# pachyderm-io/pfs

Hardware: AMD Instinct MI355X
Metric: GiB/s device-resident CDC rolling-hash + chunk content-hash (higher is better)
Workload: dtype u8

## Files before the change

### pfs_amd/csrc/cdc_kernels.hip

```cpp
#include <hip/hip_runtime.h>
#include <stdint.h>
#include <stdlib.h>

#include <algorithm>
#include <type_traits>

#define PFSCDC_HD __host__ __device__
#include "index_parse.h"
#include "pfscdc_internal.h"

#define PFS_DEV __device__ __forceinline__

namespace pfscdc {


PFS_DEV uint64_t rotl1_64(uint64_t x) { return (x << 1) | (x >> 63); }

PFS_DEV uint32_t tab_addr(uint32_t w, uint32_t lane_off, int j) {
  return __builtin_amdgcn_perm(w, lane_off, 0x0c0c0000u | ((4u + (uint32_t)j) << 8));
}

template <typename T>
PFS_DEV T lds_load(const uint8_t* lds, uint32_t byte_addr) {
  return *reinterpret_cast<const T*>(lds + byte_addr);
// ... 614 lines not shown
    }
    uint64_t total;
    const uint64_t ex = block_exscan<BLOCK>(e, s_wave, &total) + carry;
    if (t < ntiles) {
      const uint64_t ts = t * kTile;
      if (c <= (uint32_t)kTileK) {
        uint32_t o[kTileK];
#pragma unroll
        for (int i = 0; i < kTileK; i++) o[i] = i < (int)c ? recs[t].off[i] : ~0u;
#pragma unroll
        for (int i = 0; i < kTileK; i++) {
          uint32_t rank = 0;
#pragma unroll
          for (int j = 0; j < kTileK; j++) rank += o[j] < o[i];
          if (i < (int)c) entries[ex + rank] = ts + o[i];
        }
      } else {
        const uint64_t te = (ts + kTile < n) ? ts + kTile : n;
        entries[ex] = kDenseBit | (te - 1);
      }
    }
    carry += total;
  }
  if (threadIdx.x == 0) *n_entries = carry;
}

__global__ __launch_bounds__(kCompactBlock) void compact_kernel(
    const TileRec* __restrict__ recs, uint64_t ntiles, uint64_t n,
    uint64_t* __restrict__ entries, uint64_t* __restrict__ n_entries) {
  __shared__ uint64_t s_wave[kCompactBlock / 64 + 1];
  compact_tiles<kCompactBlock>(recs, ntiles, n, entries, n_entries, s_wave);
}

template <int BLOCK>
PFS_DEV uint64_t segcompact_block(const pfscdc_segment* __restrict__ slots,
                                  const uint64_t* __restrict__ seg_base,
                                  const uint64_t* __restrict__ nseg, uint32_t nfiles,
                                  pfscdc_segment* __restrict__ segs,
                                  uint64_t* __restrict__ seg_begin, uint64_t* s_wave) {
  uint64_t carry = 0;
  for (uint64_t base = 0; base < nfiles; base += BLOCK) {
    const uint64_t f = base + threadIdx.x;
    const uint64_t c = f < nfiles ? nseg[f] : 0;
    uint64_t total;
    const uint64_t ex = block_exscan<BLOCK>(c, s_wave, &total) + carry;
    if (f < nfiles) {
      seg_begin[f] = ex;
      const pfscdc_segment* src = slots + seg_base[f];
      for (uint64_t i = 0; i < c; i++) segs[ex + i] = src[i];
    }
    carry += total;
  }
  if (threadIdx.x == 0) seg_begin[nfiles] = carry;
  return carry;
}

PFS_DEV uint32_t lpt_key(uint64_t size) {
  const uint64_t nblk = (size + 127) / 128;
  const uint64_t k = nblk >> 6;
  return 1023u - (uint32_t)(k < 1023 ? k : 1023);
}

template <int BLOCK>
PFS_DEV void lpt_order_block(const pfscdc_segment* __restrict__ segs, uint64_t n,
                             uint32_t* __restrict__ order, uint32_t* __restrict__ counter,
                             uint32_t* hist, uint64_t* s_wave,
                             const uint64_t* __restrict__ offs = nullptr, uint64_t bin_bytes = 0,
                             uint32_t* __restrict__ next = nullptr, uint64_t* qlen = nullptr) {
  const bool bins = next && offs && bin_bytes;
  auto binned = [&](uint64_t i) {
    const uint32_t f = segs[i].file;
    return bins && offs[f + 1] - offs[f] <= bin_bytes;
  };
  auto entry = [&](uint64_t i, uint32_t& key) {
    if (binned(i)) {
      const uint32_t f = segs[i].file;
      key = lpt_key(offs[f + 1] - offs[f]);
      return i == 0 || segs[i - 1].file != f;
    }
    key = lpt_key(segs[i].size);
    return true;
  };
  constexpr int kPer = 1024 / BLOCK;
  static_assert(1024 % BLOCK == 0, "bins split evenly over the block");
  for (int b = 0; b < kPer; b++) hist[threadIdx.x * kPer + b] = 0;
  __syncthreads();
  for (uint64_t i = threadIdx.x; i < n; i += BLOCK) {
    uint32_t key;
    if (entry(i, key)) atomicAdd(&hist[key], 1u);
    if (bins) next[i] = binned(i) && i + 1 < n && segs[i + 1].file == segs[i].file
                            ? (uint32_t)(i + 1) : kNoNext;
  }
  __syncthreads();
  uint32_t local[kPer];
  uint64_t sum = 0;
  for (int b = 0; b < kPer; b++) {
    local[b] = hist[threadIdx.x * kPer + b];
    sum += local[b];
  }
  uint64_t total;
  uint64_t start = block_exscan<BLOCK>(sum, s_wave, &total);
  for (int b = 0; b < kPer; b++) {
    hist[threadIdx.x * kPer + b] = (uint32_t)start;
    start += local[b];
  }
  __syncthreads();
  for (uint64_t i = threadIdx.x; i < n; i += BLOCK) {
    uint32_t key;
    if (entry(i, key)) order[atomicAdd(&hist[key], 1u)] = (uint32_t)i;
  }
  if (threadIdx.x == 0) {
    *counter = 0;
    if (qlen) *qlen = total;
  }
}


PFS_DEV uint64_t rescan_first(const uint8_t* __restrict__ data, const uint64_t* __restrict__ T,
                              uint64_t a, uint64_t b, uint64_t mask) {
  const uint32_t lane = threadIdx.x & 63u;
  constexpr uint64_t W = 256;
  for (uint64_t base = a; base <= b; base += 64 * W) {
    const uint64_t st = base + lane * W;
    const uint64_t en = (st + W - 1 < b) ? st + W - 1 : b;
    uint64_t found = kNone;
    if (st <= en) {
      uint64_t h = 0;
      for (int k = 0; k < 64; k++) h = rotl1_64(h) ^ T[data[st - 63 + k]];
      if ((h & mask) == 0) found = st;
      for (uint64_t i = st + 1; found == kNone && i <= en; i++) {
        h = rotl1_64(h) ^ T[data[i - 64]] ^ T[data[i]];
        if ((h & mask) == 0) found = i;
      }
    }
    found = wave_min_u64(found);
    if (found != kNone) return found;
  }
  return kNone;
}

PFS_DEV void select_file(
    const uint8_t* __restrict__ data, const uint64_t* __restrict__ T,
    const uint64_t* __restrict__ entries, const uint64_t* __restrict__ n_entries,
    const uint64_t* __restrict__ offs, const uint64_t* __restrict__ seg_base, uint64_t f,
    uint64_t mask, uint64_t min_chunk, uint64_t max_chunk,
    pfscdc_segment* __restrict__ slots, uint64_t* __restrict__ nseg) {
  const uint32_t lane = threadIdx.x & 63u;
  const uint64_t fs = offs[f], fe = offs[f + 1];
  const uint64_t sb = seg_base[f], cap = seg_base[f + 1] - sb;
  const uint64_t ne = *n_entries;
  pfscdc_segment* out = slots + sb;
  uint64_t count = 0;
  auto emit = [&](uint64_t s, uint64_t size, uint32_t flags) {
    if (lane == 0 && count < cap) {
      out[count].offset = s - fs;
      out[count].size = size;
      out[count].file = (uint32_t)f;
      out[count].flags = flags;
    }
    count++;
  };
  uint64_t k = 0;
  {
    const uint64_t key = fs + min_chunk - 1;
    uint64_t lo = 0, hi = ne;
    while (hi - lo > 64) {
      const uint64_t step = (hi - lo + 63) / 64;
      const uint64_t i = lo + lane * step;
      const bool below = i < hi && (entries[i] & ~kDenseBit) < key;
      const uint32_t cnt = (uint32_t)__popcll(__ballot(below));
      if (cnt == 0) {
        hi = lo;
      } else {
        const uint64_t top = lo + (uint64_t)cnt * step;
        lo = lo + (uint64_t)(cnt - 1) * step + 1;
        hi = top < hi ? top : hi;
      }
    }
    const uint64_t i = lo + lane;
    const bool below = i < hi && (entries[i] & ~kDenseBit) < key;
    k = lo + (uint64_t)__popcll(__ballot(below));
  }
  uint64_t s = fs;
  while (true) {
    const uint64_t lo = s + min_chunk - 1;
    if (lo >= fe) break;
    const uint64_t hi = s + max_chunk - 1;
    const uint64_t limit = hi < fe - 1 ? hi : fe - 1;
    while (k < ne && (entries[k] & ~kDenseBit) < lo) k++;
    uint64_t c = kNone;
    for (uint64_t kk = k; kk < ne; kk++) {
      const uint64_t e = entries[kk];
      const uint64_t v = e & ~kDenseBit;
      if (!(e & kDenseBit)) {
        if (v <= limit) c = v;
        break;
      }
      const uint64_t ts = (v / kTile) * kTile;
      const uint64_t a = lo > ts ? lo : ts;
      const uint64_t bnd = v < limit ? v : limit;
      if (a <= bnd) {
        c = rescan_first(data, T, a, bnd, mask);
        if (c != kNone) break;
      }
      if (v >= limit) break;
    }
    uint64_t cut;
    if (c != kNone) cut = c;
    else if (hi <= fe - 1) cut = hi;
    else break;
    emit(s, cut + 1 - s, PFSCDC_SEG_VALID | PFSCDC_SEG_CUT);
    s = cut + 1;
  }
  if (s < fe) emit(s, fe - s, PFSCDC_SEG_VALID);
  if (lane == 0) {
    for (uint64_t i = count; i < cap; i++) out[i].flags = 0;
    nseg[f] = count;
  }
}

__global__ __launch_bounds__(kSelectBlock) void select_kernel(
    const uint8_t* __restrict__ data, const uint64_t* __restrict__ T,
    const uint64_t* __restrict__ entries, const uint64_t* __restrict__ n_entries,
    const uint64_t* __restrict__ offs, const uint64_t* __restrict__ seg_base, uint32_t nfiles,
    uint64_t mask, uint64_t min_chunk, uint64_t max_chunk,
    pfscdc_segment* __restrict__ slots, uint64_t* __restrict__ nseg, uint32_t* done_ctr,
    pfscdc_segment* __restrict__ segs, uint64_t* __restrict__ seg_begin,
    uint32_t* __restrict__ order, uint32_t* __restrict__ counter, uint64_t bin_bytes,
    uint32_t* __restrict__ next, uint64_t* __restrict__ qlen) {
  __shared__ uint32_t hist[1024];
  __shared__ uint64_t s_wave[kSelectBlock / 64 + 1];
  __shared__ uint32_t s_flag;
  const uint64_t f = ((uint64_t)blockIdx.x * kSelectBlock + threadIdx.x) >> 6;
  if (f < nfiles)
    select_file(data, T, entries, n_entries, offs, seg_base, f, mask, min_chunk, max_chunk,
                slots, nseg);
  if (!last_block_done(done_ctr, &s_flag)) return;
  const uint64_t total = segcompact_block<kSelectBlock>(slots, seg_base, nseg, nfiles, segs,
                                                        seg_begin, s_wave);
  __threadfence_block();
  __syncthreads();
  if (order)
    lpt_order_block<kSelectBlock>(segs, total, order, counter, hist, s_wave, offs, bin_bytes,
                                  next, qlen);
}


__global__ __launch_bounds__(kCompactBlock) void segcompact_kernel(
    const pfscdc_segment* __restrict__ slots, const uint64_t* __restrict__ seg_base,
    const uint64_t* __restrict__ nseg, uint32_t nfiles, pfscdc_segment* __restrict__ segs,
    uint64_t* __restrict__ seg_begin) {
  __shared__ uint64_t s_wave[kCompactBlock / 64 + 1];
  segcompact_block<kCompactBlock>(slots, seg_base, nseg, nfiles, segs, seg_begin, s_wave);
}

__global__ __launch_bounds__(kCompactBlock) void hash_order_kernel(
    const pfscdc_segment* __restrict__ segs, const uint64_t* __restrict__ seg_count,
    uint32_t* __restrict__ order, uint32_t* __restrict__ counter) {
  __shared__ uint32_t hist[1024];
  __shared__ uint64_t s_wave[kCompactBlock / 64 + 1];
  lpt_order_block<kCompactBlock>(segs, *seg_count, order, counter, hist, s_wave);
}


constexpr uint64_t kB2IV[8] = {
    0x6a09e667f3bcc908ULL, 0xbb67ae8584caa73bULL, 0x3c6ef372fe94f82bULL,
    0xa54ff53a5f1d36f1ULL, 0x510e527fade682d1ULL, 0x9b05688c2b3e6c1fULL,
    0x1f83d9abfb41bd6bULL, 0x5be0cd19137e2179ULL};

template <typename T>
PFS_DEV T pick4(uint32_t j, T v0, T v1, T v2, T v3) {
  return j == 0 ? v0 : j == 1 ? v1 : j == 2 ? v2 : v3;
}

constexpr uint32_t kSigmaPack[12][4] = {
#define PK(a, b, c, d) ((uint32_t)(a) * 8u | (uint32_t)(b) * 8u << 8 | (uint32_t)(c) * 8u << 16 | (uint32_t)(d) * 8u << 24)
#define ROW(s0, s1, s2, s3, s4, s5, s6, s7, s8, s9, s10, s11, s12, s13, s14, s15) \
  {PK(s0, s1, s14, s15), PK(s2, s3, s8, s9), PK(s4, s5, s10, s11), PK(s6, s7, s12, s13)}
    ROW(0, 1, 2, 3, 4, 5, 6, 7, 8, 9, 10, 11, 12, 13, 14, 15),
    ROW(14, 10, 4, 8, 9, 15, 13, 6, 1, 12, 0, 2, 11, 7, 5, 3),
    ROW(11, 8, 12, 0, 5, 2, 15, 13, 10, 14, 3, 6, 7, 1, 9, 4),
    ROW(7, 9, 3, 1, 13, 12, 11, 14, 2, 6, 5, 10, 4, 0, 15, 8),
    ROW(9, 0, 5, 7, 2, 4, 10, 15, 14, 1, 11, 12, 6, 8, 3, 13),
    ROW(2, 12, 6, 10, 0, 11, 8, 3, 4, 13, 7, 5, 15, 14, 1, 9),
    ROW(12, 5, 1, 15, 14, 13, 4, 10, 0, 7, 6, 3, 9, 2, 8, 11),
    ROW(13, 11, 7, 14, 12, 1, 3, 9, 5, 0, 15, 4, 8, 6, 2, 10),
    ROW(6, 15, 14, 9, 11, 3, 0, 8, 12, 2, 13, 7, 1, 4, 10, 5),
// ... 1010 lines not shown
  scan_skip_kernel<<<grid, 256, 0, st>>>(offs, nfiles, n, min_chunk, nunits, skip,
                                         (unsigned long long*)scanned, uinfo, plan);
  hipError_t e = hipGetLastError();
  if (e != hipSuccess) return e;
  scan_slots_kernel<<<grid, 256, 0, st>>>(nunits, uinfo, plan, slots, hdr, d_hdr);
  return hipGetLastError();
}

hipError_t launch_scan(const uint8_t* data, const uint8_t* tail, uint64_t n, const uint64_t* d_table,
                       uint32_t average_bits, uint64_t ntiles, TileRec* recs, int grid,
                       uint32_t* unit_ctr, uint32_t* done_ctr, uint64_t* entries,
                       uint64_t* n_entries, uint64_t* span, hipStream_t st, const uint32_t* skip,
                       const ScanPlan* d_plan) {
  const size_t lds = kScanLdsBytes;
  const uint64_t mask64 = average_bits >= 64 ? ~0ULL : ((1ULL << average_bits) - 1);
  const ScanPlan* const pl = d_plan;
  if (average_bits <= 32)
    cdc_scan_kernel<false><<<grid, kScanBlock, lds, st>>>(
        data, tail, n, d_table, 32 - average_bits, mask64, ntiles, recs, unit_ctr, done_ctr,
        entries, n_entries, skip, span, pl);
  else
    cdc_scan_kernel<true><<<grid, kScanBlock, lds, st>>>(
        data, tail, n, d_table, 64 - average_bits, mask64, ntiles, recs, unit_ctr, done_ctr,
        entries, n_entries, skip, span, pl);
  return hipGetLastError();
}

hipError_t launch_compact(const TileRec* recs, uint64_t ntiles, uint64_t n, uint64_t* entries,
                          uint64_t* n_entries, hipStream_t st) {
  compact_kernel<<<1, kCompactBlock, 0, st>>>(recs, ntiles, n, entries, n_entries);
  return hipGetLastError();
}

hipError_t launch_select(const uint8_t* data, const uint64_t* d_table, const uint64_t* entries,
                         const uint64_t* n_entries, const uint64_t* offs,
                         const uint64_t* seg_base, uint32_t nfiles, uint32_t average_bits,
                         uint64_t min_chunk, uint64_t max_chunk, pfscdc_segment* slots,
                         uint64_t* nseg, uint32_t* done_ctr, pfscdc_segment* segs,
                         uint64_t* seg_begin, uint32_t* order, uint32_t* counter,
                         hipStream_t st, uint64_t bin_bytes, uint32_t* next, uint64_t* qlen) {
  const uint64_t mask64 = average_bits >= 64 ? ~0ULL : ((1ULL << average_bits) - 1);
  const uint64_t waves_per_block = kSelectBlock / 64;
  const uint64_t grid = (nfiles + waves_per_block - 1) / waves_per_block;
  select_kernel<<<(unsigned)grid, kSelectBlock, 0, st>>>(data, d_table, entries, n_entries,
                                                         offs, seg_base, nfiles, mask64,
                                                         min_chunk, max_chunk, slots, nseg,
                                                         done_ctr, segs, seg_begin, order,
                                                         counter, bin_bytes, next, qlen);
  return hipGetLastError();
}

hipError_t launch_segcompact(const pfscdc_segment* slots, const uint64_t* seg_base,
                             const uint64_t* nseg, uint32_t nfiles, pfscdc_segment* segs,
                             uint64_t* seg_begin, hipStream_t st) {
  segcompact_kernel<<<1, kCompactBlock, 0, st>>>(slots, seg_base, nseg, nfiles, segs, seg_begin);
  return hipGetLastError();
}

static uint32_t prio_arg(uint32_t prio) {
  return prio == kHashPrioNone ? 0u : prio ? prio : kHashPrioAuto;
}

int hash_waves(uint64_t longest_bytes, uint64_t total_bytes, int num_cus, int forced) {
  if (forced >= 1 && forced <= 8) return forced;
  const uint64_t quads1 = (uint64_t)num_cus * 4 * (64 / 4);
  const uint64_t longest = (longest_bytes + 127) / 128, total = total_bytes / 128;
  return longest * quads1 >= total ? 1 : kHashWavesPerSimd;
}

static unsigned capped_grid(uint64_t grid, Knob cap_knob) {
  const int64_t cap = knob(cap_knob);
  if (cap > 0 && (uint64_t)cap < grid) grid = (uint64_t)cap;
  return (unsigned)grid;
}

static unsigned hash_grid(uint64_t max_segments, int num_cus, int waves) {
  const uint64_t quads_per_block = kHashBlock / 4;
  const uint64_t need = (max_segments + quads_per_block - 1) / quads_per_block;
  const uint64_t full = (uint64_t)num_cus * 4 * (waves > 0 ? waves : kHashWavesPerSimd) /
                        (kHashBlock / 64);
  return capped_grid(need < full ? need : full, Knob::HashGrid);
}

hipError_t launch_blake2b(const uint8_t* data, const uint64_t* offs, pfscdc_segment* segs,
                          const uint64_t* seg_count, uint64_t max_segments, uint32_t* order,
                          uint32_t* counter, int num_cus, uint64_t nbytes, hipStream_t st,
                          bool ordered, uint64_t* span, int waves, uint32_t prio,
                          bool cu_exclusive, const uint32_t* next, uint64_t* fair,
// ... 1393 lines not shown
```

### pfs_amd/csrc/pfscdc.cpp

```cpp
#include <hip/hip_runtime.h>

#include <algorithm>
#include <cstdio>
#include <cstring>
#include <string>
#include <vector>

#include <unistd.h>

#include "dev_list.h"
#include "pfscdc_internal.h"

using namespace pfscdc;

namespace {

template <typename T>
struct DevBuf {
  T* p = nullptr;
  size_t cap = 0;
  hipError_t ensure(size_t n, bool exact = false) {
    if (n <= cap && p) return hipSuccess;
    if (p) (void)hipFree(p);
    p = nullptr;
// ... 34 lines not shown
};

struct CreatePending {
  bool active = false, split = false;
  uint32_t k = 0, nr = 0;
  uint8_t* hashes = nullptr;
  pfscdc_ref* refs = nullptr;
};

}

struct pfscdc_ctx {
  pfscdc_params params{};
  int device = 0;
  int num_cus = 256;
  hipStream_t own_stream = nullptr;
  hipStream_t stream = nullptr;
  std::string err;
  uint64_t table[256];
  uint64_t* d_table = nullptr;
  DevBuf<uint8_t> d_data, d_tail;
  DevBuf<TileRec> d_recs;
  DevBuf<uint32_t> d_unit_ctr;
  DevBuf<uint32_t> d_skip;
  DevBuf<uint32_t> d_uinfo, d_plan;
  DevBuf<uint4> d_uslots;
  DevBuf<uint32_t> d_rslots;
  DevBuf<ScanPlan> d_planhdr;
  bool scan_skipped = false;
  uint32_t scan_mode = 0;
  uint64_t scanned_bytes = 0;
  bool cuts_only = false;
  DevBuf<uint64_t> d_entries, d_counts;
  DevBuf<uint64_t> d_offs, d_seg_base, d_nseg, d_seg_begin;
  DevBuf<pfscdc_segment> d_slots, d_segs;
  DevBuf<uint32_t> d_order, d_qctr;
  DevBuf<uint32_t> d_next;
  DevBuf<pfscdc_ref> d_refs;
  DevBuf<uint8_t> d_out;
  DevBuf<uint64_t> d_span;
  PinnedBuf<uint64_t> h_span;
  double wall_khz = 100000.0;
  DevBuf<uint32_t> d_ids;
  DevBuf<uint64_t> d_starts;
  DevBuf<uint8_t> d_group, d_group_ct;
  DevBuf<pfscdc_segment> d_segs2;
  DevBuf<uint64_t> d_blk;
  DevBuf<uint8_t> d_ctext;
  PinnedBuf<uint64_t> h_blk;
  PinnedBuf<pfscdc_segment> h_segs2;
  PinnedBuf<pfscdc_ref> h_refs;
  DevBuf<pfscdc_slice> d_rslices;
  DevBuf<uint64_t> d_rmeta;
  DevBuf<uint8_t> d_rok;
  PinnedBuf<pfscdc_slice> h_rslices;
  PinnedBuf<uint64_t> h_rmeta;
  PinnedBuf<uint8_t> h_rok;
  DevBuf<TarEntry> d_tar;
  DevBuf<uint8_t> d_tnames;
  PinnedBuf<TarEntry> h_tar;
  PinnedBuf<uint8_t> h_tnames;
  hipEvent_t rev[4] = {nullptr, nullptr, nullptr, nullptr};
  float read_ms[2] = {0.f, 0.f};
  float frame_ms = 0.f;
  uint32_t options = 0;
  float get_ms = 0.f;
// ... 397 lines not shown
  if (!file_offsets) return fail(c, PFSCDC_EINVAL, "file_offsets is NULL");
  if (nbytes && !bytes) return fail(c, PFSCDC_EINVAL, "bytes is NULL");
  if (file_offsets[0] != 0 || file_offsets[nfiles] != nbytes)
    return fail(c, PFSCDC_EINVAL, "file_offsets must start at 0 and end at nbytes");
  for (uint32_t f = 0; f < nfiles; f++)
    if (file_offsets[f + 1] < file_offsets[f])
      return fail(c, PFSCDC_EINVAL, "file_offsets must be nondecreasing");
  if (bytes_on_device && ((uintptr_t)bytes & 15))
    return fail(c, PFSCDC_EINVAL, "device bytes must be 16-byte aligned");
  c->ntiles = (nbytes + kTile - 1) / kTile;
  if (c->ntiles * (uint64_t)kScanWaves >= (1ull << 32))
    return fail(c, PFSCDC_EUNSUPPORTED, "batch too large for one scan (split it)");
  c->scan_valid = false;
  HIP_OK(c, hipSetDevice(c->device));
  hipStream_t st = c->stream;
  const pfscdc_params& p = c->params;

  HIP_OK(c, c->h_offs.ensure(nfiles + 1));
  HIP_OK(c, c->h_seg_base.ensure(nfiles + 1));
  std::memcpy(c->h_offs.p, file_offsets, sizeof(uint64_t) * (nfiles + 1));
  uint64_t cap = 0, longest_file = 0;
  for (uint32_t f = 0; f < nfiles; f++) {
    c->h_seg_base.p[f] = cap;
    const uint64_t len = file_offsets[f + 1] - file_offsets[f];
    cap += len ? len / (uint64_t)p.min_chunk + 1 : 0;
    longest_file = std::max(longest_file, len);
  }
  const int waves = knob_waves(std::min<uint64_t>(longest_file, (uint64_t)p.max_chunk), nbytes,
                              c->num_cus);
  const uint64_t quads = (uint64_t)c->num_cus * 4 * (uint64_t)waves * 16;
  const int64_t kb = knob(Knob::HashBinBytes);
  const uint64_t bin_bytes = kb >= 0 ? (uint64_t)kb : (nbytes + quads - 1) / quads;
  c->h_seg_base.p[nfiles] = cap;
  c->slot_cap = cap;
  c->nfiles = nfiles;
  c->nbytes = nbytes;

  HIP_OK(c, c->d_offs.ensure(nfiles + 1));
  HIP_OK(c, c->d_seg_base.ensure(nfiles + 1));
  HIP_OK(c, c->d_nseg.ensure(nfiles + 1));
  HIP_OK(c, c->d_seg_begin.ensure(nfiles + 1));
  HIP_OK(c, c->d_slots.ensure(cap));
  HIP_OK(c, c->d_segs.ensure(cap));
  HIP_OK(c, c->d_order.ensure(cap));
  if (bin_bytes) HIP_OK(c, c->d_next.ensure(cap));
  HIP_OK(c, c->d_qctr.ensure(2));
  if (options & PFSCDC_OPT_REF_IDS) HIP_OK(c, c->d_refs.ensure(cap));
  HIP_OK(c, c->d_recs.ensure(c->ntiles));
  HIP_OK(c, c->d_unit_ctr.ensure(3));
  HIP_OK(c, c->d_entries.ensure(c->ntiles * kTileK + 1));
  HIP_OK(c, c->d_counts.ensure(7));
  HIP_OK(c, c->d_tail.ensure(kTailBytes));
  HIP_OK(c, c->d_span.ensure(kSpanSlots));
  HIP_OK(c, c->h_span.ensure(kSpanSlots + 4));

  const uint8_t* data;
  if (bytes_on_device) {
    data = (const uint8_t*)bytes;
  } else {
    HIP_OK(c, c->d_data.ensure(nbytes + 64));
    if (nbytes) HIP_OK(c, hipMemcpyAsync(c->d_data.p, bytes, nbytes, hipMemcpyHostToDevice, st));
    data = c->d_data.p;
  }
  c->dev_data = data;
  HIP_OK(c, hipMemcpyAsync(c->d_offs.p, c->h_offs.p, sizeof(uint64_t) * (nfiles + 1),
                           hipMemcpyHostToDevice, st));
  HIP_OK(c, hipMemcpyAsync(c->d_seg_base.p, c->h_seg_base.p, sizeof(uint64_t) * (nfiles + 1),
                           hipMemcpyHostToDevice, st));
  const uint64_t n_main = nbytes & ~63ULL;
  HIP_OK(c, hipMemsetAsync(c->d_tail.p, 0, kTailBytes, st));
  if (nbytes > n_main)
    HIP_OK(c, hipMemcpyAsync(c->d_tail.p, data + n_main, nbytes - n_main,
                             hipMemcpyDeviceToDevice, st));
  HIP_OK(c, hipMemsetAsync(c->d_counts.p, 0, 7 * sizeof(uint64_t), st));
  if (c->ntiles) HIP_OK(c, hipMemsetAsync(c->d_recs.p, 0, sizeof(TileRec) * c->ntiles, st));
  HIP_OK(c, hipMemsetAsync(c->d_unit_ctr.p, 0, 3 * sizeof(uint32_t), st));
  HIP_OK(c, reset_spans(c, st));

  HIP_OK(c, hipEventRecord(c->ev[0], st));
  c->scan_skipped = false;
  c->scan_mode = 0;
  if (c->ntiles) {
    const uint32_t* skip = nullptr;
    c->scan_skipped = knob(Knob::ScanSkip) != 0;
    c->scan_mode = c->scan_skipped ? PFSCDC_SCAN_SKIPPED_FIRST_MIN : 0u;
    const ScanPlan* d_plan = nullptr;
    const uint64_t nunits = c->ntiles * kScanWaves;
    if (c->scan_skipped) {
      HIP_OK(c, c->d_skip.ensure(nunits));
      const bool cs_room = nfiles < kPlanMaxFiles &&
                           (uint64_t)nfiles * kRankSlots * sizeof(uint32_t) * 64 <= nbytes;
      if (cs_room && cut_skip_exact(p)) {
        c->scan_mode |= PFSCDC_SCAN_SKIPPED_CUTS;
        HIP_OK(c, c->d_uinfo.ensure(2 * nunits));
        HIP_OK(c, c->d_uslots.ensure(nunits));
        HIP_OK(c, c->d_plan.ensure(kPlanWords));
        HIP_OK(c, c->d_rslots.ensure((size_t)nfiles * kRankSlots));
        HIP_OK(c, hipMemsetAsync(c->d_plan.p, 0, kPlanWords * sizeof(uint32_t), st));
        HIP_OK(c, hipMemsetAsync(c->d_rslots.p, 0, (size_t)nfiles * kRankSlots * sizeof(uint32_t), st));
        HIP_OK(c, c->d_planhdr.ensure(1));
        const ScanPlan hdr{c->d_uslots.p, c->d_plan.p, c->d_uinfo.p, c->d_rslots.p, c->d_offs.p,
                           (uint64_t)p.min_chunk, (uint64_t)p.max_chunk,
                           (unsigned long long*)(c->d_counts.p + 6)};
        HIP_OK(c, launch_scan_plan(c->d_offs.p, nfiles, nbytes, (uint64_t)p.min_chunk, c->ntiles,
                                   c->d_skip.p, c->d_counts.p + 3, c->d_uinfo.p, c->d_uslots.p,
                                   c->d_plan.p, hdr, c->d_planhdr.p, st));
        d_plan = c->d_planhdr.p;
      } else {
        HIP_OK(c, launch_scan_skip(c->d_offs.p, nfiles, nbytes, (uint64_t)p.min_chunk, c->ntiles,
                                   c->d_skip.p, c->d_counts.p + 3, st));
      }
      skip = c->d_skip.p;
    }
    const int grid = scan_grid(c->ntiles, c->num_cus);
    HIP_OK(c, launch_scan(data, c->d_tail.p, nbytes, c->d_table, p.average_bits, c->ntiles,
                          c->d_recs.p, grid, c->d_unit_ctr.p, c->d_unit_ctr.p + 1,
                          c->d_entries.p, c->d_counts.p, c->d_span.p, st, skip, d_plan));
  }
  HIP_OK(c, hipEventRecord(c->ev[1], st));
  HIP_OK(c, hipEventRecord(c->ev[2], st));
  if (nfiles)
    HIP_OK(c, launch_select(data, c->d_table, c->d_entries.p, c->d_counts.p, c->d_offs.p,
                            c->d_seg_base.p, nfiles, p.average_bits, (uint64_t)p.min_chunk,
                            (uint64_t)p.max_chunk, c->d_slots.p, c->d_nseg.p,
                            c->d_unit_ctr.p + 2, c->d_segs.p, c->d_seg_begin.p, c->d_order.p,
                            c->d_qctr.p, st, bin_bytes, bin_bytes ? c->d_next.p : nullptr,
                            c->d_counts.p + 4));
  const uint64_t* qlen = c->d_counts.p + 4;
  const uint32_t* next = bin_bytes ? c->d_next.p : nullptr;
  HIP_OK(c, hipEventRecord(c->ev[3], st));
  if (c->hash_after && c->hash_after->device == c->device)
    HIP_OK(c, hipStreamWaitEvent(st, c->hash_after->ev[4], 0));
  if (nfiles && !(options & kScanNoHash))
    HIP_OK(c, launch_blake2b(data, c->d_offs.p, c->d_segs.p, qlen, cap,
                             c->d_order.p, c->d_qctr.p, c->num_cus, nbytes, st, true,
                             c->d_span.p + 2, waves, 0u, waves == 1, next,
                             knob(Knob::HashFair) && waves > 1 && next ? c->d_counts.p + 5
                                                                      : nullptr,
                             (uint32_t)knob(Knob::HashFairEvery)));
  HIP_OK(c, hipEventRecord(c->ev[4], st));
  c->have_refs = (options & PFSCDC_OPT_REF_IDS) != 0 && !(options & kScanNoHash);
  if (c->have_refs && nfiles)
    HIP_OK(c, launch_ref_ids(data, c->d_offs.p, c->d_segs.p, qlen, cap,
                             c->d_order.p, c->d_qctr.p + 1, c->num_cus, nbytes, c->d_refs.p,
                             nullptr, st, waves, 0u, next, c->d_seg_begin.p + nfiles));
  HIP_OK(c, hipEventRecord(c->ev[6], st));
  HIP_OK(c, c->h_seg_begin.ensure(nfiles + 1));
  if (nfiles)
    HIP_OK(c, hipMemcpyAsync(c->h_seg_begin.p, c->d_seg_begin.p, sizeof(uint64_t) * (nfiles + 1),
                             hipMemcpyDeviceToHost, st));
  else
    c->h_seg_begin.p[0] = 0;
  c->pending = true;
  return PFSCDC_OK;
}
// ... 87 lines not shown
  if (rc) return rc;
  return pfscdc_wait(c);
}

uint64_t pfscdc_num_segments(const pfscdc_ctx* c) { return c ? c->nsegs : 0; }

int pfscdc_set_options(pfscdc_ctx* c, uint32_t options) {
  if (!c || (options & ~(PFSCDC_OPT_REF_IDS | PFSCDC_OPT_CUTS_ONLY | PFSCDC_OPT_CTEXT_IN_PLACE)))
    return PFSCDC_EINVAL;
  if (c->pending) return fail(c, PFSCDC_ESTATE, "set_options during a pending scan");
  c->options = options;
  return PFSCDC_OK;
}

const pfscdc_ref* pfscdc_refs(const pfscdc_ctx* c) {
  return c && c->have_refs && !c->pending && c->host_records ? c->h_refs.p : nullptr;
}

int pfscdc_last_ref_ms(pfscdc_ctx* c, float* ms) {
  if (!c || !ms) return PFSCDC_EINVAL;
  *ms = 0.f;
  if (c->have_refs) PFS_HIP(c, hipEventElapsedTime(ms, c->ev[4], c->ev[6]));
  return PFSCDC_OK;
}
const pfscdc_segment* pfscdc_segments(const pfscdc_ctx* c) {
  return c && c->host_records ? c->h_segs.p : nullptr;
}
const uint64_t* pfscdc_file_segment_begin(const pfscdc_ctx* c) {
  return c ? c->h_seg_begin.p : nullptr;
}

uint64_t pfscdc_debug_candidates(pfscdc_ctx* c, uint64_t* out, uint64_t cap) {
  if (!c || c->pending || !c->ntiles) return 0;
  uint64_t ne = 0;
  if (hipMemcpy(&ne, c->d_counts.p, sizeof ne, hipMemcpyDeviceToHost) != hipSuccess) return 0;
  if (out && cap) {
    const uint64_t k = std::min(ne, cap);
    if (hipMemcpy(out, c->d_entries.p, k * sizeof(uint64_t), hipMemcpyDeviceToHost) != hipSuccess)
      return 0;
  }
  return ne;
}

int pfscdc_last_scan_bytes(pfscdc_ctx* c, uint64_t* out) {
  if (!c || !out) return PFSCDC_EINVAL;
  if (c->pending) return fail(c, PFSCDC_ESTATE, "scan pending");
  *out = c->scanned_bytes;
  return PFSCDC_OK;
}

int pfscdc_last_scan_mode(pfscdc_ctx* c, uint32_t* mode) {
  if (!c || !mode) return PFSCDC_EINVAL;
  if (c->pending) return fail(c, PFSCDC_ESTATE, "scan pending");
  *mode = c->scan_mode;
  return PFSCDC_OK;
}

int pfscdc_last_timings(pfscdc_ctx* c, float out[5]) {
  if (!c || !out) return PFSCDC_EINVAL;
  PFS_HIP(c, hipEventElapsedTime(&out[0], c->ev[0], c->ev[1]));
  PFS_HIP(c, hipEventElapsedTime(&out[1], c->ev[1], c->ev[2]));
  PFS_HIP(c, hipEventElapsedTime(&out[2], c->ev[2], c->ev[3]));
  PFS_HIP(c, hipEventElapsedTime(&out[3], c->ev[3], c->ev[4]));
  PFS_HIP(c, hipEventElapsedTime(&out[4], c->ev[0], c->ev[4]));
  return PFSCDC_OK;
}
// ... 319 lines not shown
  return PFSCDC_OK;
}

int pfscdc_candidates(pfscdc_ctx* c, const void* bytes, uint64_t nbytes, int bytes_on_device,
                      uint64_t halo, uint64_t* out, uint64_t cap, uint64_t* n) {
  if (!c || !n || (cap && !out) || (nbytes && !bytes)) return PFSCDC_EINVAL;
  *n = 0;
  if (c->pending) return fail(c, PFSCDC_ESTATE, "candidates during a pending scan");
  if (int rc = check_device_arg(c, bytes, bytes_on_device, "bytes")) return rc;
  if (halo > 64) return fail(c, PFSCDC_EINVAL, "halo must be at most 64 bytes");
  const uint64_t ntiles = (nbytes + kTile - 1) / kTile;
  if (ntiles * (uint64_t)kScanWaves >= (1ull << 32))
    return fail(c, PFSCDC_EUNSUPPORTED, "range too large for one scan (split it)");
  if (nbytes <= halo) return PFSCDC_OK;
  scan_overwritten(c);
  PFS_HIP(c, hipSetDevice(c->device));
  hipStream_t st = c->stream;
  PFS_HIP(c, c->d_recs.ensure(ntiles));
  PFS_HIP(c, c->d_unit_ctr.ensure(3));
  PFS_HIP(c, c->d_entries.ensure(ntiles * kTileK + 1));
  PFS_HIP(c, c->d_counts.ensure(4));
  PFS_HIP(c, c->d_tail.ensure(kTailBytes));
  PFS_HIP(c, c->d_span.ensure(kSpanSlots));
  const uint8_t* data;
  PFS_HIP(c, stage_in(c, bytes, nbytes, bytes_on_device, st, &data));
  const uint64_t n_main = nbytes & ~63ULL;
  PFS_HIP(c, hipMemsetAsync(c->d_tail.p, 0, kTailBytes, st));
  if (nbytes > n_main)
    PFS_HIP(c, hipMemcpyAsync(c->d_tail.p, data + n_main, nbytes - n_main,
                              hipMemcpyDeviceToDevice, st));
  PFS_HIP(c, hipMemsetAsync(c->d_counts.p, 0, 4 * sizeof(uint64_t), st));
  PFS_HIP(c, hipMemsetAsync(c->d_recs.p, 0, sizeof(TileRec) * ntiles, st));
  PFS_HIP(c, hipMemsetAsync(c->d_unit_ctr.p, 0, 3 * sizeof(uint32_t), st));
  PFS_HIP(c, reset_spans(c, st));
  PFS_HIP(c, hipEventRecord(c->ev[0], st));
  const int grid = scan_grid(ntiles, c->num_cus);
  PFS_HIP(c, launch_scan(data, c->d_tail.p, nbytes, c->d_table, c->params.average_bits, ntiles,
                         c->d_recs.p, grid, c->d_unit_ctr.p, c->d_unit_ctr.p + 1, c->d_entries.p,
                         c->d_counts.p, c->d_span.p, st));
  PFS_HIP(c, hipEventRecord(c->ev[1], st));
  PFS_HIP(c, hipEventRecord(c->ev[2], st));
  uint64_t ne = 0;
  PFS_HIP(c, hipMemcpyAsync(&ne, c->d_counts.p, sizeof ne, hipMemcpyDeviceToHost, st));
  PFS_HIP(c, hipStreamSynchronize(st));
  std::vector<uint64_t> ent(ne);
  if (ne)
    PFS_HIP(c, hipMemcpy(ent.data(), c->d_entries.p, ne * sizeof(uint64_t), hipMemcpyDeviceToHost));
  const uint64_t mask = c->params.average_bits >= 64 ? ~0ULL
                                                     : ((1ULL << c->params.average_bits) - 1);
  std::vector<uint8_t> win;
  uint64_t k = 0;
  auto emit = [&](uint64_t p) {
    if (p < halo) return;
    if (k < cap) out[k] = p;
    k++;
  };
  for (uint64_t e : ent) {
    if (!(e & kDenseBit)) {
      emit(e);
      continue;
    }
    const uint64_t te = e & ~kDenseBit, ts = (te / kTile) * kTile;
    const uint64_t a = ts >= 64 ? ts - 64 : 0;
    win.resize(te + 1 - a);
    PFS_HIP(c, hipMemcpy(win.data(), data + a, win.size(), hipMemcpyDeviceToHost));
    auto byte = [&](uint64_t p) -> uint64_t { return p >= a ? win[p - a] : 0; };
// ... 657 lines not shown
```

### pfs_amd/csrc/pfscdc_internal.h

```cpp
#pragma once
#include <hip/hip_runtime.h>
#include <stdint.h>

#include <string>
#include <vector>

#include "../../include/pfscdc.h"

namespace pfscdc {

constexpr int kScanWaves = 12;
constexpr int kScanBlock = 64 * kScanWaves;
constexpr int kStrip = 4096;
constexpr uint64_t kTile = (uint64_t)kScanBlock * kStrip;
constexpr int kTileK = 15;
constexpr uint32_t kTableLdsBytes = 256u * 256u;
constexpr uint32_t kStageBytes = 64u * 128u;
constexpr uint32_t kScanLdsBytes = kTableLdsBytes + kScanWaves * kStageBytes;
static_assert(kScanLdsBytes <= 160 * 1024, "scan kernel LDS budget");
constexpr int kCompactBlock = 1024;
constexpr int kSelectBlock = 1024;
constexpr int kHashBlock = 256;
constexpr int kHashWavesPerSimd = 2;
constexpr uint64_t kDenseBit = 1ULL << 63;
// ... 55 lines not shown

hipError_t prepare_kernels();

constexpr uint64_t kScanUnit = 64ull * kStrip;
constexpr uint64_t kUnitStep = 64ull * 128;
constexpr uint32_t kUnitSteps = kStrip / 128;
constexpr uint32_t kPlanBuckets = 64;
constexpr uint32_t kPlanWords = 2 + kPlanBuckets;
constexpr uint32_t kPlanMaxFiles = 1u << 24;
constexpr uint32_t kRankSlots = 64;
constexpr uint32_t kSlotDone = 1u << 31;
struct ScanPlan {
  const uint4* slots;
  const uint32_t* plan;
  const uint32_t* uinfo;
  uint32_t* rslots;
  const uint64_t* offs;
  uint64_t min_chunk, max_chunk;
  unsigned long long* dyn_skipped;
};
hipError_t launch_scan(const uint8_t* data, const uint8_t* tail, uint64_t n, const uint64_t* d_table,
                       uint32_t average_bits, uint64_t ntiles, TileRec* recs, int grid,
                       uint32_t* unit_ctr, uint32_t* done_ctr, uint64_t* entries,
                       uint64_t* n_entries, uint64_t* span, hipStream_t st,
                       const uint32_t* skip = nullptr, const ScanPlan* d_plan = nullptr);
hipError_t launch_scan_skip(const uint64_t* offs, uint32_t nfiles, uint64_t n, uint64_t min_chunk,
                            uint64_t ntiles, uint32_t* skip, uint64_t* scanned, hipStream_t st);
hipError_t launch_scan_plan(const uint64_t* offs, uint32_t nfiles, uint64_t n, uint64_t min_chunk,
                            uint64_t ntiles, uint32_t* skip, uint64_t* scanned, uint32_t* uinfo,
                            uint4* slots, uint32_t* plan, const ScanPlan& hdr, ScanPlan* d_hdr,
                            hipStream_t st);
hipError_t launch_compact(const TileRec* recs, uint64_t ntiles, uint64_t n, uint64_t* entries,
                          uint64_t* n_entries, hipStream_t st);
hipError_t launch_select(const uint8_t* data, const uint64_t* d_table, const uint64_t* entries,
                         const uint64_t* n_entries, const uint64_t* offs,
                         const uint64_t* seg_base, uint32_t nfiles, uint32_t average_bits,
                         uint64_t min_chunk, uint64_t max_chunk, pfscdc_segment* slots,
                         uint64_t* nseg, uint32_t* done_ctr, pfscdc_segment* segs,
                         uint64_t* seg_begin, uint32_t* order, uint32_t* counter,
                         hipStream_t st, uint64_t bin_bytes = 0, uint32_t* next = nullptr,
                         uint64_t* qlen = nullptr);
hipError_t launch_segcompact(const pfscdc_segment* slots, const uint64_t* seg_base,
                             const uint64_t* nseg, uint32_t nfiles, pfscdc_segment* segs,
                             uint64_t* seg_begin, hipStream_t st);
constexpr uint32_t kHashPrioAuto = 0x3fffffffu;
constexpr uint32_t kHashPrioNone = 0x80000000u;
hipError_t launch_blake2b(const uint8_t* data, const uint64_t* offs, pfscdc_segment* segs,
                          const uint64_t* seg_count, uint64_t max_segments, uint32_t* order,
                          uint32_t* counter, int num_cus, uint64_t nbytes, hipStream_t st,
                          bool ordered = false, uint64_t* span = nullptr, int waves = 0,
                          uint32_t prio = 0,
                          bool cu_exclusive = false,
                          const uint32_t* next = nullptr,
                          uint64_t* fair = nullptr,
                          uint32_t fair_every = 256);
int hash_waves(uint64_t longest_bytes, uint64_t total_bytes, int num_cus, int forced);
hipError_t launch_order(const pfscdc_segment* segs, const uint64_t* seg_count, uint32_t* order,
                        uint32_t* counter, hipStream_t st);
hipError_t launch_ref_ids(const uint8_t* data, const uint64_t* offs, pfscdc_segment* segs,
                          const uint64_t* seg_count, uint64_t max_segments, const uint32_t* order,
                          uint32_t* counter, int num_cus, uint64_t nbytes, pfscdc_ref* refs,
                          uint8_t* ctext_out, hipStream_t st, int waves = 0, uint32_t prio = 0,
                          const uint32_t* next = nullptr,
                          const uint64_t* nsegs = nullptr);
hipError_t launch_deks(pfscdc_segment* segs, const uint64_t* seg_count, uint64_t max_segments,
                       pfscdc_ref* refs, uint32_t* counter, hipStream_t st);
hipError_t launch_chacha_xor(const uint8_t* data, const uint64_t* offs, const pfscdc_segment* segs,
                             const uint64_t* blk_base, uint32_t n, uint64_t nblocks,
                             const pfscdc_ref* refs, uint8_t* out, int num_cus, hipStream_t st,
                             bool prio = false, bool one_wave_per_simd = false);
hipError_t launch_get(const uint8_t* ctext, const uint64_t* offs, pfscdc_segment* segs,
                      const uint64_t* seg_count, uint64_t nsegs, uint32_t* order, uint32_t* counter,
                      int num_cus, uint64_t nbytes, pfscdc_ref* refs, uint8_t* ptext, hipStream_t st,
                      int waves = 0);
hipError_t launch_verify_ids(const pfscdc_segment* segs, uint32_t n, const pfscdc_ref* refs,
                             uint8_t* ok, hipStream_t st);
hipError_t launch_slice_gather(const uint8_t* ctext, const uint64_t* chunk_offs,
// ... 262 lines not shown
```

Measured before the change: 1393.

## Replace serial segment compaction with decoupled look-back scan in select kernel

```diff
diff --git a/pfs_amd/csrc/cdc_kernels.hip b/pfs_amd/csrc/cdc_kernels.hip
--- a/pfs_amd/csrc/cdc_kernels.hip
+++ b/pfs_amd/csrc/cdc_kernels.hip
@@ -670,36 +670,13 @@
   compact_tiles<kCompactBlock>(recs, ntiles, n, entries, n_entries, s_wave);
 }
 
-template <int BLOCK>
-PFS_DEV uint64_t segcompact_block(const pfscdc_segment* __restrict__ slots,
-                                  const uint64_t* __restrict__ seg_base,
-                                  const uint64_t* __restrict__ nseg, uint32_t nfiles,
-                                  pfscdc_segment* __restrict__ segs,
-                                  uint64_t* __restrict__ seg_begin, uint64_t* s_wave) {
-  uint64_t carry = 0;
-  for (uint64_t base = 0; base < nfiles; base += BLOCK) {
-    const uint64_t f = base + threadIdx.x;
-    const uint64_t c = f < nfiles ? nseg[f] : 0;
-    uint64_t total;
-    const uint64_t ex = block_exscan<BLOCK>(c, s_wave, &total) + carry;
-    if (f < nfiles) {
-      seg_begin[f] = ex;
-      const pfscdc_segment* src = slots + seg_base[f];
-      for (uint64_t i = 0; i < c; i++) segs[ex + i] = src[i];
-    }
-    carry += total;
-  }
-  if (threadIdx.x == 0) seg_begin[nfiles] = carry;
-  return carry;
-}
-
 PFS_DEV uint32_t lpt_key(uint64_t size) {
   const uint64_t nblk = (size + 127) / 128;
   const uint64_t k = nblk >> 6;
   return 1023u - (uint32_t)(k < 1023 ? k : 1023);
 }
 
-template <int BLOCK>
+template <int BLOCK, bool HAVE_HIST = false>
 PFS_DEV void lpt_order_block(const pfscdc_segment* __restrict__ segs, uint64_t n,
                              uint32_t* __restrict__ order, uint32_t* __restrict__ counter,
                              uint32_t* hist, uint64_t* s_wave,
@@ -721,13 +698,15 @@
   };
   constexpr int kPer = 1024 / BLOCK;
   static_assert(1024 % BLOCK == 0, "bins split evenly over the block");
-  for (int b = 0; b < kPer; b++) hist[threadIdx.x * kPer + b] = 0;
-  __syncthreads();
-  for (uint64_t i = threadIdx.x; i < n; i += BLOCK) {
-    uint32_t key;
-    if (entry(i, key)) atomicAdd(&hist[key], 1u);
-    if (bins) next[i] = binned(i) && i + 1 < n && segs[i + 1].file == segs[i].file
-                            ? (uint32_t)(i + 1) : kNoNext;
+  if (!HAVE_HIST) {
+    for (int b = 0; b < kPer; b++) hist[threadIdx.x * kPer + b] = 0;
+    __syncthreads();
+    for (uint64_t i = threadIdx.x; i < n; i += BLOCK) {
+      uint32_t key;
+      if (entry(i, key)) atomicAdd(&hist[key], 1u);
+      if (bins) next[i] = binned(i) && i + 1 < n && segs[i + 1].file == segs[i].file
+                              ? (uint32_t)(i + 1) : kNoNext;
+    }
   }
   __syncthreads();
   uint32_t local[kPer];
@@ -777,16 +756,52 @@
   return kNone;
 }
 
-PFS_DEV void select_file(
+PFS_DEV uint64_t first_candidate(const uint8_t* __restrict__ data, const uint64_t* __restrict__ T,
+                                 const TileRec* __restrict__ recs, uint64_t n, uint64_t lo,
+                                 uint64_t limit, uint64_t mask) {
+  const uint32_t lane = threadIdx.x & 63u;
+  const uint64_t t1 = limit / kTile;
+  uint64_t t = lo / kTile;
+  while (t <= t1) {
+    const uint64_t tl = t + lane;
+    const uint32_t cl = tl <= t1 ? recs[tl].count : 0u;
+    const uint64_t some = __ballot(cl != 0);
+    if (!some) {
+      t += 64;
+      continue;
+    }
+    const uint32_t j = (uint32_t)__builtin_ctzll(some);
+    t += j;
+    const uint32_t c = (uint32_t)__builtin_amdgcn_readlane((int)cl, (int)j);
+    const uint64_t ts = t * kTile;
+    if (c <= (uint32_t)kTileK) {
+      uint64_t v = lane < c ? ts + recs[t].off[lane] : kNone;
+      if (v < lo) v = kNone;
+      v = wave_min_u64(v);
+      if (v != kNone) return v <= limit ? v : kNone;
+    } else {
+      const uint64_t te = (ts + kTile < n) ? ts + kTile : n;
+      const uint64_t a = lo > ts ? lo : ts;
+      const uint64_t bnd = te - 1 < limit ? te - 1 : limit;
+      if (a <= bnd) {
+        const uint64_t v = rescan_first(data, T, a, bnd, mask);
+        if (v != kNone) return v;
+      }
+    }
+    t++;
+  }
+  return kNone;
+}
+
+PFS_DEV uint64_t select_file(
     const uint8_t* __restrict__ data, const uint64_t* __restrict__ T,
-    const uint64_t* __restrict__ entries, const uint64_t* __restrict__ n_entries,
+    const TileRec* __restrict__ recs, uint64_t n,
     const uint64_t* __restrict__ offs, const uint64_t* __restrict__ seg_base, uint64_t f,
     uint64_t mask, uint64_t min_chunk, uint64_t max_chunk,
     pfscdc_segment* __restrict__ slots, uint64_t* __restrict__ nseg) {
   const uint32_t lane = threadIdx.x & 63u;
   const uint64_t fs = offs[f], fe = offs[f + 1];
   const uint64_t sb = seg_base[f], cap = seg_base[f + 1] - sb;
-  const uint64_t ne = *n_entries;
   pfscdc_segment* out = slots + sb;
   uint64_t count = 0;
   auto emit = [&](uint64_t s, uint64_t size, uint32_t flags) {
@@ -798,51 +813,13 @@
     }
     count++;
   };
-  uint64_t k = 0;
-  {
-    const uint64_t key = fs + min_chunk - 1;
-    uint64_t lo = 0, hi = ne;
-    while (hi - lo > 64) {
-      const uint64_t step = (hi - lo + 63) / 64;
-      const uint64_t i = lo + lane * step;
-      const bool below = i < hi && (entries[i] & ~kDenseBit) < key;
-      const uint32_t cnt = (uint32_t)__popcll(__ballot(below));
-      if (cnt == 0) {
-        hi = lo;
-      } else {
-        const uint64_t top = lo + (uint64_t)cnt * step;
-        lo = lo + (uint64_t)(cnt - 1) * step + 1;
-        hi = top < hi ? top : hi;
-      }
-    }
-    const uint64_t i = lo + lane;
-    const bool below = i < hi && (entries[i] & ~kDenseBit) < key;
-    k = lo + (uint64_t)__popcll(__ballot(below));
-  }
   uint64_t s = fs;
   while (true) {
     const uint64_t lo = s + min_chunk - 1;
     if (lo >= fe) break;
     const uint64_t hi = s + max_chunk - 1;
     const uint64_t limit = hi < fe - 1 ? hi : fe - 1;
-    while (k < ne && (entries[k] & ~kDenseBit) < lo) k++;
-    uint64_t c = kNone;
-    for (uint64_t kk = k; kk < ne; kk++) {
-      const uint64_t e = entries[kk];
-      const uint64_t v = e & ~kDenseBit;
-      if (!(e & kDenseBit)) {
-        if (v <= limit) c = v;
-        break;
-      }
-      const uint64_t ts = (v / kTile) * kTile;
-      const uint64_t a = lo > ts ? lo : ts;
-      const uint64_t bnd = v < limit ? v : limit;
-      if (a <= bnd) {
-        c = rescan_first(data, T, a, bnd, mask);
-        if (c != kNone) break;
-      }
-      if (v >= limit) break;
-    }
+    const uint64_t c = first_candidate(data, T, recs, n, lo, limit, mask);
     uint64_t cut;
     if (c != kNone) cut = c;
     else if (hi <= fe - 1) cut = hi;
@@ -855,42 +832,136 @@
     for (uint64_t i = count; i < cap; i++) out[i].flags = 0;
     nseg[f] = count;
   }
-}
-
-__global__ __launch_bounds__(kSelectBlock) void select_kernel(
+  return count;
+}
+
+PFS_DEV uint64_t wave_sum_u64(uint64_t v) {
+#pragma unroll
+  for (int o = 32; o > 0; o >>= 1) {
+    const uint32_t lo = __shfl_xor((uint32_t)v, o, 64);
+    const uint32_t hi = __shfl_xor((uint32_t)(v >> 32), o, 64);
+    v += ((uint64_t)hi << 32) | lo;
+  }
+  return v;
+}
+
+constexpr uint64_t kPartOwn = 1ULL << 62;
+constexpr uint64_t kPartIncl = 1ULL << 63;
+constexpr uint64_t kPartMask = kPartOwn - 1;
+constexpr uint32_t kPartField = 31;
+constexpr int kSelectWavesPerEu = 6;
+
+__global__ __launch_bounds__(kSelectBlock) __attribute__((amdgpu_waves_per_eu(kSelectWavesPerEu, kSelectWavesPerEu))) void select_kernel(
     const uint8_t* __restrict__ data, const uint64_t* __restrict__ T,
-    const uint64_t* __restrict__ entries, const uint64_t* __restrict__ n_entries,
+    const TileRec* __restrict__ recs, uint64_t n,
     const uint64_t* __restrict__ offs, const uint64_t* __restrict__ seg_base, uint32_t nfiles,
     uint64_t mask, uint64_t min_chunk, uint64_t max_chunk,
     pfscdc_segment* __restrict__ slots, uint64_t* __restrict__ nseg, uint32_t* done_ctr,
+    uint32_t* ticket_ctr, uint32_t* ghist, uint64_t* part,
     pfscdc_segment* __restrict__ segs, uint64_t* __restrict__ seg_begin,
     uint32_t* __restrict__ order, uint32_t* __restrict__ counter, uint64_t bin_bytes,
     uint32_t* __restrict__ next, uint64_t* __restrict__ qlen) {
+  constexpr int kWaves = kSelectBlock / 64;
+  constexpr int kPer = 1024 / kSelectBlock;
+  static_assert(kWaves <= 64 && 1024 % kSelectBlock == 0, "one wave scans the block's waves");
   __shared__ uint32_t hist[1024];
-  __shared__ uint64_t s_wave[kSelectBlock / 64 + 1];
-  __shared__ uint32_t s_flag;
-  const uint64_t f = ((uint64_t)blockIdx.x * kSelectBlock + threadIdx.x) >> 6;
-  if (f < nfiles)
-    select_file(data, T, entries, n_entries, offs, seg_base, f, mask, min_chunk, max_chunk,
-                slots, nseg);
-  if (!last_block_done(done_ctr, &s_flag)) return;
-  const uint64_t total = segcompact_block<kSelectBlock>(slots, seg_base, nseg, nfiles, segs,
-                                                        seg_begin, s_wave);
-  __threadfence_block();
+  __shared__ uint64_t s_wave[kWaves + 1];
+  __shared__ uint64_t s_own[kWaves];
+  __shared__ uint64_t s_base;
+  __shared__ uint32_t s_flag, s_ticket;
+  if (threadIdx.x == 0) s_ticket = atomicAdd(ticket_ctr, 1u);
+  for (int b = 0; b < kPer; b++) hist[threadIdx.x * kPer + b] = 0;
+  __syncthreads();
+  const uint32_t vb = s_ticket;
+  const uint32_t lane = threadIdx.x & 63u, wave = threadIdx.x >> 6;
+  const uint64_t f = (uint64_t)vb * kWaves + wave;
+  const bool bins = next && bin_bytes;
+  uint64_t count = 0, fsize = 0;
+  bool binned = false;
+  if (f < nfiles) {
+    count = select_file(data, T, recs, n, offs, seg_base, f, mask, min_chunk, max_chunk, slots,
+                        nseg);
+    fsize = offs[f + 1] - offs[f];
+    binned = bins && fsize <= bin_bytes;
+  }
+  const uint64_t entries = binned ? (count ? 1 : 0) : count;
+  if (lane == 0) s_own[wave] = count | entries << kPartField;
+  __syncthreads();
+  if (wave == 0) {
+    const uint64_t own = wave_sum_u64(lane < kWaves ? s_own[lane] : 0);
+    if (lane == 0)
+      __hip_atomic_store(part + vb, kPartOwn | own, __ATOMIC_RELAXED, __HIP_MEMORY_SCOPE_AGENT);
+    uint64_t base = 0;
+    for (int64_t pos = vb; pos > 0; pos -= 64) {
+      const int64_t i = pos - 1 - (int64_t)lane;
+      uint64_t w = 0;
+      if (i >= 0) {
+        while (!((w = __hip_atomic_load(part + i, __ATOMIC_RELAXED, __HIP_MEMORY_SCOPE_AGENT)) >>
+                 62))
+          __builtin_amdgcn_s_sleep(1);
+      }
+      const uint64_t incl = __ballot((w & kPartIncl) != 0);
+      const uint32_t stop = incl ? (uint32_t)__builtin_ctzll(incl) : 64u;
+      base += wave_sum_u64(lane <= stop ? w & kPartMask : 0);
+      if (incl) break;
+    }
+    if (lane == 0) {
+      __hip_atomic_store(part + vb, kPartIncl | (base + own), __ATOMIC_RELAXED,
+                         __HIP_MEMORY_SCOPE_AGENT);
+      s_base = base;
+      if (vb == gridDim.x - 1) seg_begin[nfiles] = (base + own) & ((1ULL << kPartField) - 1);
+    }
+  }
+  __syncthreads();
+  if (f < nfiles) {
+    uint64_t at = s_base;
+    for (uint32_t w = 0; w < wave; w++) at += s_own[w];
+    const uint64_t sbeg = at & ((1ULL << kPartField) - 1), ebeg = at >> kPartField;
+    if (lane == 0) seg_begin[f] = sbeg;
+    const pfscdc_segment* src = slots + seg_base[f];
+    for (uint64_t i = lane; i < count; i += 64) {
+      const pfscdc_segment sg = src[i];
+      segs[sbeg + i] = sg;
+      if (bins) next[sbeg + i] = binned && i + 1 < count ? (uint32_t)(sbeg + i + 1) : kNoNext;
+      if (order && !binned) {
+        atomicAdd(&hist[lpt_key(sg.size)], 1u);
+        order[ebeg + i] = (uint32_t)(sbeg + i);
+      }
+    }
+    if (order && binned && count && lane == 0) {
+      atomicAdd(&hist[lpt_key(fsize)], 1u);
+      order[ebeg] = (uint32_t)sbeg;
+    }
+  }
   __syncthreads();
   if (order)
-    lpt_order_block<kSelectBlock>(segs, total, order, counter, hist, s_wave, offs, bin_bytes,
-                                  next, qlen);
-}
-
-
-__global__ __launch_bounds__(kCompactBlock) void segcompact_kernel(
-    const pfscdc_segment* __restrict__ slots, const uint64_t* __restrict__ seg_base,
-    const uint64_t* __restrict__ nseg, uint32_t nfiles, pfscdc_segment* __restrict__ segs,
-    uint64_t* __restrict__ seg_begin) {
-  __shared__ uint64_t s_wave[kCompactBlock / 64 + 1];
-  segcompact_block<kCompactBlock>(slots, seg_base, nseg, nfiles, segs, seg_begin, s_wave);
-}
+    for (int b = 0; b < kPer; b++) {
+      const uint32_t h = hist[threadIdx.x * kPer + b];
+      if (h) atomicAdd(&ghist[threadIdx.x * kPer + b], h);
+    }
+  if (!last_block_done(done_ctr, &s_flag)) return;
+  if (!order) return;
+  uint64_t sum = 0, used = 0;
+  for (int b = 0; b < kPer; b++) {
+    const uint32_t h = ghist[threadIdx.x * kPer + b];
+    hist[threadIdx.x * kPer + b] = h;
+    sum += h;
+    used += h != 0;
+  }
+  uint64_t total, keys;
+  block_exscan<kSelectBlock>(used, s_wave, &keys);
+  if (keys <= 1) {
+    block_exscan<kSelectBlock>(sum, s_wave, &total);
+    if (threadIdx.x == 0) {
+      *counter = 0;
+      if (qlen) *qlen = total;
+    }
+    return;
+  }
+  lpt_order_block<kSelectBlock, true>(segs, seg_begin[nfiles], order, counter, hist, s_wave,
+                                      offs, bin_bytes, next, qlen);
+}
+
 
 __global__ __launch_bounds__(kCompactBlock) void hash_order_kernel(
     const pfscdc_segment* __restrict__ segs, const uint64_t* __restrict__ seg_count,
@@ -1967,28 +2038,23 @@
   return hipGetLastError();
 }
 
-hipError_t launch_select(const uint8_t* data, const uint64_t* d_table, const uint64_t* entries,
-                         const uint64_t* n_entries, const uint64_t* offs,
+uint64_t select_blocks(uint32_t nfiles) {
+  const uint64_t waves_per_block = kSelectBlock / 64;
+  return (nfiles + waves_per_block - 1) / waves_per_block;
+}
+
+hipError_t launch_select(const uint8_t* data, const uint64_t* d_table, const TileRec* recs,
+                         uint64_t n, const uint64_t* offs,
                          const uint64_t* seg_base, uint32_t nfiles, uint32_t average_bits,
                          uint64_t min_chunk, uint64_t max_chunk, pfscdc_segment* slots,
-                         uint64_t* nseg, uint32_t* done_ctr, pfscdc_segment* segs,
+                         uint64_t* nseg, uint32_t* sel_words, pfscdc_segment* segs,
                          uint64_t* seg_begin, uint32_t* order, uint32_t* counter,
                          hipStream_t st, uint64_t bin_bytes, uint32_t* next, uint64_t* qlen) {
   const uint64_t mask64 = average_bits >= 64 ? ~0ULL : ((1ULL << average_bits) - 1);
-  const uint64_t waves_per_block = kSelectBlock / 64;
-  const uint64_t grid = (nfiles + waves_per_block - 1) / waves_per_block;
-  select_kernel<<<(unsigned)grid, kSelectBlock, 0, st>>>(data, d_table, entries, n_entries,
-                                                         offs, seg_base, nfiles, mask64,
-                                                         min_chunk, max_chunk, slots, nseg,
-                                                         done_ctr, segs, seg_begin, order,
-                                                         counter, bin_bytes, next, qlen);
-  return hipGetLastError();
-}
-
-hipError_t launch_segcompact(const pfscdc_segment* slots, const uint64_t* seg_base,
-                             const uint64_t* nseg, uint32_t nfiles, pfscdc_segment* segs,
-                             uint64_t* seg_begin, hipStream_t st) {
-  segcompact_kernel<<<1, kCompactBlock, 0, st>>>(slots, seg_base, nseg, nfiles, segs, seg_begin);
+  select_kernel<<<(unsigned)select_blocks(nfiles), kSelectBlock, 0, st>>>(
+      data, d_table, recs, n, offs, seg_base, nfiles, mask64, min_chunk, max_chunk, slots, nseg,
+      sel_words, sel_words + 1, sel_words + kSelHist, (uint64_t*)(sel_words + kSelPart), segs,
+      seg_begin, order, counter, bin_bytes, next, qlen);
   return hipGetLastError();
 }
 
diff --git a/pfs_amd/csrc/pfscdc.cpp b/pfs_amd/csrc/pfscdc.cpp
--- a/pfs_amd/csrc/pfscdc.cpp
+++ b/pfs_amd/csrc/pfscdc.cpp
@@ -90,6 +90,7 @@
   uint64_t scanned_bytes = 0;
   bool cuts_only = false;
   DevBuf<uint64_t> d_entries, d_counts;
+  bool entries_deferred = false;
   DevBuf<uint64_t> d_offs, d_seg_base, d_nseg, d_seg_begin;
   DevBuf<pfscdc_segment> d_slots, d_segs;
   DevBuf<uint32_t> d_order, d_qctr;
@@ -553,6 +554,8 @@
   const int64_t kb = knob(Knob::HashBinBytes);
   const uint64_t bin_bytes = kb >= 0 ? (uint64_t)kb : (nbytes + quads - 1) / quads;
   c->h_seg_base.p[nfiles] = cap;
+  if (cap >= (1ull << 31))
+    return fail(c, PFSCDC_EUNSUPPORTED, "batch too large for one scan (split it)");
   c->slot_cap = cap;
   c->nfiles = nfiles;
   c->nbytes = nbytes;
@@ -568,7 +571,8 @@
   HIP_OK(c, c->d_qctr.ensure(2));
   if (options & PFSCDC_OPT_REF_IDS) HIP_OK(c, c->d_refs.ensure(cap));
   HIP_OK(c, c->d_recs.ensure(c->ntiles));
-  HIP_OK(c, c->d_unit_ctr.ensure(3));
+  const size_t ctr_words = 2 + select_words(nfiles);
+  HIP_OK(c, c->d_unit_ctr.ensure(ctr_words));
   HIP_OK(c, c->d_entries.ensure(c->ntiles * kTileK + 1));
   HIP_OK(c, c->d_counts.ensure(7));
   HIP_OK(c, c->d_tail.ensure(kTailBytes));
@@ -595,12 +599,13 @@
                              hipMemcpyDeviceToDevice, st));
   HIP_OK(c, hipMemsetAsync(c->d_counts.p, 0, 7 * sizeof(uint64_t), st));
   if (c->ntiles) HIP_OK(c, hipMemsetAsync(c->d_recs.p, 0, sizeof(TileRec) * c->ntiles, st));
-  HIP_OK(c, hipMemsetAsync(c->d_unit_ctr.p, 0, 3 * sizeof(uint32_t), st));
+  HIP_OK(c, hipMemsetAsync(c->d_unit_ctr.p, 0, ctr_words * sizeof(uint32_t), st));
   HIP_OK(c, reset_spans(c, st));
 
   HIP_OK(c, hipEventRecord(c->ev[0], st));
   c->scan_skipped = false;
   c->scan_mode = 0;
+  c->entries_deferred = c->ntiles != 0;
   if (c->ntiles) {
     const uint32_t* skip = nullptr;
     c->scan_skipped = knob(Knob::ScanSkip) != 0;
@@ -635,13 +640,13 @@
     }
     const int grid = scan_grid(c->ntiles, c->num_cus);
     HIP_OK(c, launch_scan(data, c->d_tail.p, nbytes, c->d_table, p.average_bits, c->ntiles,
-                          c->d_recs.p, grid, c->d_unit_ctr.p, c->d_unit_ctr.p + 1,
-                          c->d_entries.p, c->d_counts.p, c->d_span.p, st, skip, d_plan));
+                          c->d_recs.p, grid, c->d_unit_ctr.p, nullptr, c->d_entries.p,
+                          c->d_counts.p, c->d_span.p, st, skip, d_plan));
   }
   HIP_OK(c, hipEventRecord(c->ev[1], st));
   HIP_OK(c, hipEventRecord(c->ev[2], st));
   if (nfiles)
-    HIP_OK(c, launch_select(data, c->d_table, c->d_entries.p, c->d_counts.p, c->d_offs.p,
+    HIP_OK(c, launch_select(data, c->d_table, c->d_recs.p, nbytes, c->d_offs.p,
                             c->d_seg_base.p, nfiles, p.average_bits, (uint64_t)p.min_chunk,
                             (uint64_t)p.max_chunk, c->d_slots.p, c->d_nseg.p,
                             c->d_unit_ctr.p + 2, c->d_segs.p, c->d_seg_begin.p, c->d_order.p,
@@ -795,6 +800,14 @@
 
 uint64_t pfscdc_debug_candidates(pfscdc_ctx* c, uint64_t* out, uint64_t cap) {
   if (!c || c->pending || !c->ntiles) return 0;
+  if (c->entries_deferred) {
+    if (hipSetDevice(c->device) != hipSuccess ||
+        launch_compact(c->d_recs.p, c->ntiles, c->nbytes, c->d_entries.p, c->d_counts.p,
+                       c->stream) != hipSuccess ||
+        hipStreamSynchronize(c->stream) != hipSuccess)
+      return 0;
+    c->entries_deferred = false;
+  }
   uint64_t ne = 0;
   if (hipMemcpy(&ne, c->d_counts.p, sizeof ne, hipMemcpyDeviceToHost) != hipSuccess) return 0;
   if (out && cap) {
@@ -1180,6 +1193,7 @@
   PFS_HIP(c, hipMemsetAsync(c->d_counts.p, 0, 4 * sizeof(uint64_t), st));
   PFS_HIP(c, hipMemsetAsync(c->d_recs.p, 0, sizeof(TileRec) * ntiles, st));
   PFS_HIP(c, hipMemsetAsync(c->d_unit_ctr.p, 0, 3 * sizeof(uint32_t), st));
+  c->entries_deferred = false;
   PFS_HIP(c, reset_spans(c, st));
   PFS_HIP(c, hipEventRecord(c->ev[0], st));
   const int grid = scan_grid(ntiles, c->num_cus);
diff --git a/pfs_amd/csrc/pfscdc_internal.h b/pfs_amd/csrc/pfscdc_internal.h
--- a/pfs_amd/csrc/pfscdc_internal.h
+++ b/pfs_amd/csrc/pfscdc_internal.h
@@ -111,17 +111,18 @@
                             hipStream_t st);
 hipError_t launch_compact(const TileRec* recs, uint64_t ntiles, uint64_t n, uint64_t* entries,
                           uint64_t* n_entries, hipStream_t st);
-hipError_t launch_select(const uint8_t* data, const uint64_t* d_table, const uint64_t* entries,
-                         const uint64_t* n_entries, const uint64_t* offs,
+constexpr uint32_t kSelHist = 2;
+constexpr uint32_t kSelPart = kSelHist + 1024;
+uint64_t select_blocks(uint32_t nfiles);
+inline size_t select_words(uint32_t nfiles) { return kSelPart + 2 * select_blocks(nfiles); }
+hipError_t launch_select(const uint8_t* data, const uint64_t* d_table, const TileRec* recs,
+                         uint64_t n, const uint64_t* offs,
                          const uint64_t* seg_base, uint32_t nfiles, uint32_t average_bits,
                          uint64_t min_chunk, uint64_t max_chunk, pfscdc_segment* slots,
-                         uint64_t* nseg, uint32_t* done_ctr, pfscdc_segment* segs,
+                         uint64_t* nseg, uint32_t* sel_words, pfscdc_segment* segs,
                          uint64_t* seg_begin, uint32_t* order, uint32_t* counter,
                          hipStream_t st, uint64_t bin_bytes = 0, uint32_t* next = nullptr,
                          uint64_t* qlen = nullptr);
-hipError_t launch_segcompact(const pfscdc_segment* slots, const uint64_t* seg_base,
-                             const uint64_t* nseg, uint32_t nfiles, pfscdc_segment* segs,
-                             uint64_t* seg_begin, hipStream_t st);
 constexpr uint32_t kHashPrioAuto = 0x3fffffffu;
 constexpr uint32_t kHashPrioNone = 0x80000000u;
 hipError_t launch_blake2b(const uint8_t* data, const uint64_t* offs, pfscdc_segment* segs,
```

Result: no change. 1405 (median of 6 runs) (+0.8%).
